# arkworks-rs/pcd

Measured on AMD Instinct MI355X. Metric: msm_mscalar_mul_per_s, higher is better.
Workload: dtype u32 (11 x 28-bit unsaturated Montgomery limbs, v_mad_u64_u32 with 64-bit column accumulators); 1 GPU; MNT4-298 G1 variable-base MSM, n=1048576 pairs per GPU (2^20 per GPU), proving-key bases and scalars resident in HBM, scalar distribution uniform; curve=MNT4-298, group=G1, log_n=20, window_bits=20, windows=15

## Files before the change

### pcd_amd/csrc/ec.hip.h

```cpp
#pragma once
#include <type_traits>
#include "fp.hip.h"

namespace pcd {

template <class F>
struct Jac {
  F X, Y, Z;
  PCD_HD static Jac infinity() { return {F::zero(), F::one(), F::zero()}; }
  PCD_HD bool is_inf() const { return Z.is_zero(); }
  static constexpr int WORDS = 3 * F::WORDS;
  static constexpr int ABI_WORDS = 3 * F::ABI_WORDS;
  PCD_HD static Jac load(const uint32_t* p) { return {F::load(p), F::load(p + F::WORDS), F::load(p + 2 * F::WORDS)}; }
  PCD_HD void store(uint32_t* p) const { X.store(p); Y.store(p + F::WORDS); Z.store(p + 2 * F::WORDS); }
  PCD_HD static Jac from_abi(const uint32_t* w) { return {F::from_abi(w), F::from_abi(w + F::ABI_WORDS), F::from_abi(w + 2 * F::ABI_WORDS)}; }
  PCD_HD void to_abi(uint32_t* w) const { X.to_abi(w); Y.to_abi(w + F::ABI_WORDS); Z.to_abi(w + 2 * F::ABI_WORDS); }
};

template <class F>
struct Aff {
  F x, y;
  static constexpr int WORDS = 2 * F::WORDS;
  static constexpr int ABI_WORDS = 2 * F::ABI_WORDS;
  PCD_HD bool is_inf() const { return x.is_raw_zero() && y.is_raw_zero(); }
// ... 298 lines not shown
    return o;
  }

  struct AccLz {
    typename F::Lz X;
    F Y, ZZ, ZZZ;
    bool inf;
  };
  static constexpr int ACC_WORDS = 4 * F::WORDS;
  PCD_HD static AccLz lz_infinity() { AccLz a; a.X = F::zero().lz(); a.Y = F::one(); a.ZZ = F::zero(); a.ZZZ = F::zero(); a.inf = true; return a; }
  PCD_HD static AccLz lz_from(const J& p) {
    AccLz a;
    a.inf = p.is_inf();
    a.X = p.X.lz(); a.Y = p.Y; a.ZZ = p.Z.sqr(); a.ZZZ = a.ZZ * p.Z;
    return a;
  }
  PCD_HD static J lz_to_jac(const AccLz& a) {
    if (a.inf) return J::infinity();
    return {F::lz_mul(a.X, a.ZZ.lz()), a.Y * a.ZZZ, a.ZZ};
  }
  PCD_HD static AccLz madd_lz(const AccLz& p, const A& q) {
    typedef typename F::Lz L;
    if (q.is_inf()) return p;
    if (p.inf) { AccLz o; o.X = q.x.lz(); o.Y = q.y; o.ZZ = F::one(); o.ZZZ = F::one(); o.inf = false; return o; }
    const L zz = p.ZZ.lz(), zzz = p.ZZZ.lz();
    const F U2 = F::lz_mul(q.x.lz(), zz);
    const F S2 = F::lz_mul(q.y.lz(), zzz);
    const L P = F::lz_carry(F::template lz_sub<2>(U2.lz(), p.X));
    const L R = F::lz_carry(F::template lz_sub<0>(S2.lz(), p.Y.lz()));
    const F PP = F::lz_sqr(P);
    const F RR = F::lz_sqr(R);
    if (PP.is_zero()) {
      if (!RR.is_zero()) return lz_infinity();
      return lz_from(dbl(lz_to_jac(p)));
    }
    const L pp = PP.lz();
    const F PPP = F::lz_mul(P, pp);
    const F Q = F::lz_mul(p.X, pp);
    AccLz o;
    o.inf = false;
    {
      L t;
#pragma unroll
      for (int i = 0; i < F::N; i++)
        t.v[i] = (int32_t)RR.v[i] - (int32_t)PPP.v[i] - (int32_t)(Q.v[i] << 1) + (int32_t)(F::Params::mod4(i) << 1);
      o.X = F::lz_carry(t);
    }
    const L t2 = F::template lz_sub<2>(Q.lz(), o.X);
    const L y1n = F::template lz_sub<0>(F::zero().lz(), p.Y.lz());
    const L ppp = PPP.lz();
    o.Y = F::lz_dot2(R, t2, y1n, ppp);
    o.ZZ = F::lz_mul(zz, pp);
    o.ZZZ = F::lz_mul(zzz, ppp);
    return o;
  }

  template <class ST>
  PCD_HD static void madd_lz_st(ST& st, const A& q) {
    typedef typename F::Lz L;
    if (q.is_inf()) return;
    if (st.inf()) { st.st(0, q.x); st.st(1, q.y); st.st(2, F::one()); st.st(3, F::one()); st.inf() = false; return; }
    auto as_lz = [](const F& f) { L l;
#pragma unroll
      for (int i = 0; i < F::N; i++) l.v[i] = (int32_t)f.v[i];
      return l; };
    auto as_f = [](const L& l) { F f;
#pragma unroll
      for (int i = 0; i < F::N; i++) f.v[i] = (uint32_t)l.v[i];
      return f; };
    const F U2 = F::lz_mul(q.x.lz(), st.ld(2).lz());
    const F S2 = F::lz_mul(q.y.lz(), st.ld(3).lz());
    const L P = F::lz_carry(F::template lz_sub<2>(U2.lz(), as_lz(st.ld(0))));
    const L R = F::lz_carry(F::template lz_sub<0>(S2.lz(), st.ld(1).lz()));
    const F PP = F::lz_sqr(P);
    const F RR = F::lz_sqr(R);
    if (PP.is_zero()) {
      AccLz p;
      p.X = as_lz(st.ld(0)); p.Y = st.ld(1); p.ZZ = st.ld(2); p.ZZZ = st.ld(3); p.inf = false;
      AccLz o = RR.is_zero() ? lz_from(dbl(lz_to_jac(p))) : lz_infinity();
      st.st(0, as_f(o.X)); st.st(1, o.Y); st.st(2, o.ZZ); st.st(3, o.ZZZ); st.inf() = o.inf;
      return;
    }
    const L pp = PP.lz();
    const F PPP = F::lz_mul(P, pp);
    const F Q = F::lz_mul(as_lz(st.ld(0)), pp);
    L x3;
    {
      L t;
#pragma unroll
      for (int i = 0; i < F::N; i++)
        t.v[i] = (int32_t)RR.v[i] - (int32_t)PPP.v[i] - (int32_t)(Q.v[i] << 1) + (int32_t)(F::Params::mod4(i) << 1);
      x3 = F::lz_carry(t);
    }
    const L t2 = F::template lz_sub<2>(Q.lz(), x3);
    st.st(0, as_f(x3));
    const L ppp = PPP.lz();
    {
      const L y1n = F::template lz_sub<0>(F::zero().lz(), st.ld(1).lz());
      st.st(1, F::lz_dot2(R, t2, y1n, ppp));
    }
    st.st(2, F::lz_mul(st.ld(2).lz(), pp));
    st.st(3, F::lz_mul(st.ld(3).lz(), ppp));
  }

  PCD_HD static J mul_w4(const J& p, const uint32_t* k, int nwords, J* table) {
    table[0] = p;
// ... 177 lines not shown
```

### pcd_amd/csrc/fp.hip.h

```cpp
#pragma once
#include <hip/hip_runtime.h>
#include <stdint.h>

#if defined(__HIP_DEVICE_COMPILE__) && !defined(PCD_NO_KEEP_CHAIN)
__device__ __attribute__((weak)) int64_t pcd_never_s = INT64_MIN;
__device__ __attribute__((weak)) uint64_t pcd_never_u = UINT64_MAX;
#define PCD_KEEP_S(acc) __builtin_assume((acc) != pcd_never_s)
#if defined(PCD_KEEP_CHAIN_UNSIGNED)
#define PCD_KEEP_U(acc) __builtin_assume((acc) != pcd_never_u)
#else
#define PCD_KEEP_U(acc) do { if constexpr (N > 11) __builtin_assume((acc) != pcd_never_u); } while (0)
#endif
#if defined(PCD_KEEP_CHAIN_UNSIGNED)
#define PCD_KEEP_UM(acc) __builtin_assume((acc) != pcd_never_u)
#else
#define PCD_KEEP_UM(acc) do { if constexpr (N > 11 && INLINE_ARITH) __builtin_assume((acc) != pcd_never_u); } while (0)
#endif
#else
#define PCD_KEEP_S(acc) ((void)0)
#define PCD_KEEP_U(acc) ((void)0)
#define PCD_KEEP_UM(acc) ((void)0)
#endif


// ... 362 lines not shown
    return r; }
  PCD_HD static Fp lz_dot4(const Lz& a0, const Lz& b0, const Lz& a1, const Lz& b1, const Lz& a2, const Lz& b2, const Lz& a3, const Lz& b3) {
    int32_t m[N];
    int64_t acc = 0;
    PCD_LZ_WIDE_DECL
#pragma unroll
    for (int k = 0; k < N; k++) {
#pragma unroll
      for (int i = 0; i <= k; i++) {
        acc += (int64_t)a0.v[i] * b0.v[k - i]; PCD_KEEP_S(acc); PCD_LZ_WIDE_MAC(a0.v[i], b0.v[k - i])
        acc += (int64_t)a1.v[i] * b1.v[k - i]; PCD_KEEP_S(acc); PCD_LZ_WIDE_MAC(a1.v[i], b1.v[k - i])
        acc += (int64_t)a2.v[i] * b2.v[k - i]; PCD_KEEP_S(acc); PCD_LZ_WIDE_MAC(a2.v[i], b2.v[k - i])
        acc += (int64_t)a3.v[i] * b3.v[k - i]; PCD_KEEP_S(acc); PCD_LZ_WIDE_MAC(a3.v[i], b3.v[k - i])
      }
#pragma unroll
      for (int i = 0; i < k; i++) { acc += (int64_t)m[i] * (int32_t)P::mod(k - i); PCD_KEEP_S(acc); PCD_LZ_WIDE_MAC(m[i], P::mod(k - i)) }
      m[k] = (int32_t)(((uint32_t)acc * P::INV) & MASK);
      acc += (int64_t)m[k] * (int32_t)P::mod(0); PCD_KEEP_S(acc);
      PCD_LZ_WIDE_MAC(m[k], P::mod(0))
      PCD_LZ_WIDE_CHECK();
      acc >>= 28;
    }
    Fp r;
#pragma unroll
    for (int k = N; k < 2 * N - 1; k++) {
#pragma unroll
      for (int i = k - N + 1; i < N; i++) {
        acc += (int64_t)a0.v[i] * b0.v[k - i]; PCD_KEEP_S(acc); PCD_LZ_WIDE_MAC(a0.v[i], b0.v[k - i])
        acc += (int64_t)a1.v[i] * b1.v[k - i]; PCD_KEEP_S(acc); PCD_LZ_WIDE_MAC(a1.v[i], b1.v[k - i])
        acc += (int64_t)a2.v[i] * b2.v[k - i]; PCD_KEEP_S(acc); PCD_LZ_WIDE_MAC(a2.v[i], b2.v[k - i])
        acc += (int64_t)a3.v[i] * b3.v[k - i]; PCD_KEEP_S(acc); PCD_LZ_WIDE_MAC(a3.v[i], b3.v[k - i])
      }
#pragma unroll
      for (int i = k - N + 1; i < N; i++) { acc += (int64_t)m[i] * (int32_t)P::mod(k - i); PCD_KEEP_S(acc); PCD_LZ_WIDE_MAC(m[i], P::mod(k - i)) }
      r.v[k - N] = (uint32_t)acc & MASK;
      PCD_LZ_WIDE_CHECK();
      acc >>= 28;
    }
    if (acc < 0 || acc >= ((int64_t)1 << 28)) {
#if defined(PCD_LZ_CHECK) && !defined(__HIP_DEVICE_COMPILE__)
      abort();
#endif
    }
    r.v[N - 1] = (uint32_t)acc;
    return r;
  }
  PCD_HD static Fp lz_mul(const Lz& a, const Lz& b) { return lz_dot<1>(a, b, a, b); }
  PCD_HD static Fp lz_dot2(const Lz& a0, const Lz& b0, const Lz& a1, const Lz& b1) { return lz_dot<2>(a0, b0, a1, b1); }
  PCD_HD static Fp lz_sqr(const Lz& a) {
    int32_t m[N], a2[N];
#pragma unroll
    for (int i = 0; i < N; i++) a2[i] = a.v[i] * 2;
    int64_t acc = 0;
#pragma unroll
    for (int k = 0; k < N; k++) {
#pragma unroll
      for (int i = 0; 2 * i < k; i++) { acc += (int64_t)a2[i] * a.v[k - i]; PCD_KEEP_S(acc); }
      if ((k & 1) == 0) { acc += (int64_t)a.v[k / 2] * a.v[k / 2]; PCD_KEEP_S(acc); }
#pragma unroll
      for (int i = 0; i < k; i++) { acc += (int64_t)m[i] * (int32_t)P::mod(k - i); PCD_KEEP_S(acc); }
      m[k] = (int32_t)(((uint32_t)acc * P::INV) & MASK);
      acc += (int64_t)m[k] * (int32_t)P::mod(0); PCD_KEEP_S(acc);
      acc >>= 28;
    }
    Fp r;
#pragma unroll
    for (int k = N; k < 2 * N - 1; k++) {
#pragma unroll
      for (int i = k - N + 1; 2 * i < k; i++) { acc += (int64_t)a2[i] * a.v[k - i]; PCD_KEEP_S(acc); }
      if ((k & 1) == 0) { acc += (int64_t)a.v[k / 2] * a.v[k / 2]; PCD_KEEP_S(acc); }
#pragma unroll
      for (int i = k - N + 1; i < N; i++) { acc += (int64_t)m[i] * (int32_t)P::mod(k - i); PCD_KEEP_S(acc); }
      r.v[k - N] = (uint32_t)acc & MASK;
      acc >>= 28;
    }
    r.v[N - 1] = (uint32_t)acc;
    return r;
  }

  template <int TERMS>
  __host__ __device__ __noinline__ static void dot_call(Fp& out, const Fp& a0, const Fp& b0, const Fp& a1, const Fp& b1, const Fp& a2,
                                                        const Fp& b2) {
    dot_impl<TERMS>(out, a0, b0, a1, b1, a2, b2);
  }
  template <int TERMS>
  PCD_HD static void dot(Fp& out, const Fp& a0, const Fp& b0, const Fp& a1, const Fp& b1, const Fp& a2, const Fp& b2) {
    if constexpr (INLINE_ARITH) dot_impl<TERMS>(out, a0, b0, a1, b1, a2, b2); else dot_call<TERMS>(out, a0, b0, a1, b1, a2, b2);
  }
  template <int TERMS>
  PCD_HD static void dot_impl(Fp& out, const Fp& a0, const Fp& b0, const Fp& a1, const Fp& b1, const Fp& a2, const Fp& b2) {
    uint32_t m[N];
    uint64_t acc = 0;
#pragma unroll
    for (int k = 0; k < N; k++) {
#pragma unroll
      for (int i = 0; i <= k; i++) {
        acc += (uint64_t)a0.v[i] * b0.v[k - i]; PCD_KEEP_U(acc);
        acc += (uint64_t)a1.v[i] * b1.v[k - i]; PCD_KEEP_U(acc);
        if (TERMS == 3) { acc += (uint64_t)a2.v[i] * b2.v[k - i]; PCD_KEEP_U(acc); }
      }
#pragma unroll
      for (int i = 0; i < k; i++) { acc += (uint64_t)m[i] * P::mod(k - i); PCD_KEEP_U(acc); }
      m[k] = ((uint32_t)acc * P::INV) & MASK;
      acc += (uint64_t)m[k] * P::mod(0); PCD_KEEP_U(acc);
      acc >>= 28;
    }
    int32_t r[N];
#pragma unroll
    for (int k = N; k < 2 * N - 1; k++) {
#pragma unroll
      for (int i = k - N + 1; i < N; i++) {
        acc += (uint64_t)a0.v[i] * b0.v[k - i]; PCD_KEEP_U(acc);
        acc += (uint64_t)a1.v[i] * b1.v[k - i]; PCD_KEEP_U(acc);
        if (TERMS == 3) { acc += (uint64_t)a2.v[i] * b2.v[k - i]; PCD_KEEP_U(acc); }
      }
#pragma unroll
      for (int i = k - N + 1; i < N; i++) { acc += (uint64_t)m[i] * P::mod(k - i); PCD_KEEP_U(acc); }
      r[k - N] = (int32_t)((uint32_t)acc & MASK);
      acc >>= 28;
    }
    r[N - 1] = (int32_t)(uint32_t)acc;
    if (TERMS == 3) { out = norm_reduce<false>(r); return; }
#pragma unroll
    for (int i = 0; i < N; i++) out.v[i] = (uint32_t)r[i];
  }
  PCD_HD static Fp dot2(const Fp& a0, const Fp& b0, const Fp& a1, const Fp& b1) { Fp o; dot<2>(o, a0, b0, a1, b1, a0, a0); return o; }
// ... 484 lines not shown
```

### pcd_amd/csrc/msm.hip.h

```cpp
#pragma once
#include <cstdlib>
#include <math.h>

#include <algorithm>
#include <atomic>
#include <type_traits>
#include <vector>

#include "ec.hip.h"

namespace pcd {

template <int K>
struct EventSet {
  hipEvent_t e[K] = {};
  bool live = false;
  hipError_t create() {
    for (int i = 0; i < K; i++) { hipError_t r = hipEventCreate(&e[i]); if (r != hipSuccess) return r; }
    live = true;
    return hipSuccess;
  }
  hipEvent_t operator[](int i) const { return e[i]; }
  ~EventSet() { for (int i = 0; i < K; i++) if (e[i]) (void)hipEventDestroy(e[i]); }
};
// ... 668 lines not shown
        w.w = 4 * k + 3 < F::N ? a.v[4 * k + 3] : 0u;
        box[(slot * CH + k) * 64 + threadIdx.x] = w;
      }
    }
  };
  Store s;
  PCD_DEV MsmRunLazyLds() {
    __shared__ V4 accbox[4 * CH * 64];
    s.box = (LdsV4)accbox;
    s.is_inf = true;
  }
  PCD_DEV void add(const Aff<F>& q) { EC<G>::madd_lz_st(s, q); }
  PCD_DEV void flush(uint32_t* dst) {
    if (s.is_inf) { F::zero().store(dst + 2 * F::WORDS); return; }
    s.ld(0).store(dst); s.ld(1).store(dst + F::WORDS); s.ld(2).store(dst + 2 * F::WORDS); s.ld(3).store(dst + 3 * F::WORDS);
    s.is_inf = true;
  }
};
#endif
template <class G, bool XYZZ = MsmUseXyzz<G>::value>
struct MsmStoredPlain {
  typedef typename G::F F;
  static constexpr int WORDS = EC<G>::ACCX_WORDS;
  PCD_DEV static Jac<F> load(const uint32_t* p) {
    typename EC<G>::AccX a = {F::load(p), F::load(p + F::WORDS), F::load(p + 2 * F::WORDS), F::load(p + 3 * F::WORDS)};
    return EC<G>::x_to_jac(a);
  }
  static constexpr bool SEPARATE = true;
};
template <class G>
struct MsmStoredPlain<G, false> {
  typedef typename G::F F;
  static constexpr int WORDS = Jac<F>::WORDS;
  PCD_DEV static Jac<F> load(const uint32_t* p) { return Jac<F>::load(p); }
  static constexpr bool SEPARATE = false;
};
template <class G, bool LAZY = LazyCapable<typename G::F>::value>
struct MsmStored : MsmStoredPlain<G> {};
template <class G>
struct MsmStored<G, true> {
  typedef typename G::F F;
  static constexpr int WORDS = EC<G>::ACC_WORDS;
  PCD_DEV static Jac<F> load(const uint32_t* p) {
    typename EC<G>::AccLz a;
    a.ZZ = F::load(p + 2 * F::WORDS);
    if (a.ZZ.is_zero()) return Jac<F>::infinity();
    a.inf = false;
#pragma unroll
    for (int i = 0; i < F::N; i++) a.X.v[i] = (int32_t)p[i];
    a.Y = F::load(p + F::WORDS);
    a.ZZZ = F::load(p + 3 * F::WORDS);
    return EC<G>::lz_to_jac(a);
  }
  static constexpr bool SEPARATE = true;
};

template <class G>
struct MsmAccWaves {
  typedef typename AccOf<G>::type::F FA;
#ifndef PCD_ACC_WAVES_SPLIT
#define PCD_ACC_WAVES_SPLIT 2
#endif
#ifndef PCD_ACC_WAVES_G1
#define PCD_ACC_WAVES_G1 2
#endif
#ifndef PCD_ACC_WAVES_MB298
#define PCD_ACC_WAVES_MB298 2
#endif
  static constexpr int value = !FA::Base::INLINE_ARITH ? (FA::Base::N <= 11 ? PCD_ACC_WAVES_MB298 : 1)
                             : FA::DEG == 1 ? PCD_ACC_WAVES_G1 : AccOf<G>::LANES > 1 ? PCD_ACC_WAVES_SPLIT : 1;
};

template <class G, bool COMPACT>
__global__ void __launch_bounds__(64, MsmAccWaves<G>::value) msm_accumulate_kernel(const uint32_t* __restrict__ bases, const MsmEntrySource src,
                                                            const uint32_t* __restrict__ off, uint32_t nkeys,
                                                            uint32_t chunk, uint32_t* __restrict__ buckets,
                                                            uint32_t* __restrict__ piece_first, uint32_t* __restrict__ piece_last,
                                                            uint64_t plan ) {
  if (plan) chunk = msm_chunk_of_plan(off[nkeys], plan);
  typedef typename AccOf<G>::type GA;
  typedef typename GA::F F;
  typedef EC<GA> E;
  constexpr int RW = MsmStored<GA>::WORDS;
  constexpr uint32_t LANES = AccOf<G>::LANES, PER_WAVE = 64 / LANES;
  if (threadIdx.x >= PER_WAVE * LANES) return;
  uint32_t t = blockIdx.x * PER_WAVE + threadIdx.x / LANES;
  const uint32_t M = off[nkeys];
  uint64_t start64 = (uint64_t)t * chunk;
  if (start64 >= M) return;
  uint32_t start = (uint32_t)start64, end = (uint32_t)min((uint64_t)M, start64 + chunk);
  if (!COMPACT && src.flag && *src.flag != 0) return;
  if (COMPACT && src.flag && *src.flag == 0) return;
  MsmCursor cur;
  cur.seek(off, nkeys, start);
  bool open_start = cur.key_start < start;
#if PCD_ACC_LDS
  typename std::conditional<LazyCapable<F>::value, MsmRunLazyLds<GA>, MsmRunPlain<GA>>::type acc;
#else
  typename std::conditional<LazyCapable<F>::value, MsmRunLazy<GA>, MsmRunPlain<GA>>::type acc;
#endif
  constexpr bool PREFETCH = F::Base::INLINE_ARITH;
  const uint32_t ones_start = off[src.ones_key];
  auto point_of = [&](uint32_t e) {
    Aff<F> q = Aff<F>::load(bases + (size_t)(e & ~MSM_NEG) * MsmBaseStride<G>::value);
    const F ny = q.y.neg();
    if (e & MSM_NEG) q.y = ny;
    return q;
  };
// ... 284 lines not shown
      for (uint32_t i = 0; i < cnt; i++) {
        const uint32_t k0 = in[(size_t)(2 * i) * 64], l0 = in[(size_t)(2 * i + 1) * 64];
        if (k0 != key) {
          if (open_start) { acc.flush(piece_first + (size_t)t * RW); open_start = false; }
          else acc.flush(buckets + (size_t)key * RW);
          key = k0;
        }
        acc.add(point_of(l0));
      }
      const bool open_end = off[key + 1] > end;
      if (open_end) acc.flush(piece_last + (size_t)t * RW);
      else if (open_start) acc.flush(piece_first + (size_t)t * RW);
      else acc.flush(buckets + (size_t)key * RW);
    }
  }
}

template <class G>
struct MsmItems {
  typedef typename SplitOfTail<G>::type GA;
  static constexpr uint32_t LANES = SplitOfTail<G>::LANES, PER_WAVE = 64 / LANES;
  PCD_DEV static bool idle() { return threadIdx.x >= PER_WAVE * LANES; }
  PCD_DEV static uint32_t local() { return threadIdx.x / LANES; }
  PCD_DEV static uint32_t item() { return blockIdx.x * PER_WAVE + threadIdx.x / LANES; }
  static uint32_t grid(uint32_t items) { return (items + PER_WAVE - 1) / PER_WAVE; }
};

static __global__ void __launch_bounds__(256) msm_zero_kernel(uint32_t* __restrict__ cnt, uint32_t n_cnt, uint32_t* __restrict__ ctl4) {
  const uint32_t i = blockIdx.x * blockDim.x + threadIdx.x;
  if (i < n_cnt) cnt[i] = 0;
  if (i < 4) ctl4[i] = 0;
}

#ifndef PCD_SINGLE_ITEM_PLAIN
#define PCD_SINGLE_ITEM_PLAIN 0
#endif
template <class G> struct MsmSingleItem {
  typedef typename std::conditional<PCD_SINGLE_ITEM_PLAIN != 0, typename SplitOf<G>::type, typename SplitOfTail<G>::type>::type GA;
  static constexpr int LANES = PCD_SINGLE_ITEM_PLAIN != 0 ? SplitOf<G>::LANES : SplitOfTail<G>::LANES;
};
template <class G>
__global__ void __launch_bounds__(64) msm_merge_ones_kernel(uint32_t* __restrict__ buckets, uint32_t ones_key) {
  typedef typename MsmSingleItem<G>::GA GA;
  typedef typename GA::F F;
  if (blockIdx.x != 0 || threadIdx.x >= MsmSingleItem<G>::LANES) return;
  Jac<F> a = Jac<F>::load(buckets + (size_t)1 * Jac<F>::WORDS);
  Jac<F> b = Jac<F>::load(buckets + (size_t)ones_key * Jac<F>::WORDS);
  EC<GA>::add(a, b).store(buckets + (size_t)1 * Jac<F>::WORDS);
}

template <class G>
__global__ void __launch_bounds__(64) msm_fixup_kernel(const uint32_t* __restrict__ off, uint32_t nkeys, const MsmChunkRule rule,
                                                       const uint32_t* __restrict__ piece_first, const uint32_t* __restrict__ piece_last,
                                                       const uint32_t* __restrict__ acc_buckets ,
                                                       uint32_t* __restrict__ buckets, uint32_t big_limit, uint32_t* __restrict__ big_count,
                                                       uint32_t* __restrict__ big_list , uint32_t big_cap,
                                                       uint32_t* __restrict__ seg_list , uint32_t seg_len) {
  const uint32_t chunk = rule.eval(off, nkeys);
  typedef typename MsmItems<G>::GA GA;
  typedef typename GA::F F;
  typedef EC<GA> E;
  constexpr int RW = MsmStored<GA>::WORDS;
  if (MsmItems<G>::idle()) return;
  const bool lead = threadIdx.x % MsmItems<G>::LANES == 0;
  const uint32_t item = MsmItems<G>::item();
  if (item < 2) {
    const uint32_t key = item == 0 ? 1u : nkeys - 1;
    const uint32_t lo = off[key], hi = off[key + 1];
    if (hi == lo) F::zero().store(buckets + (size_t)key * Jac<F>::WORDS + 2 * F::WORDS);
    else if (MsmStored<GA>::SEPARATE && hi - (lo / chunk) * chunk <= chunk)
      MsmStored<GA>::load(acc_buckets + (size_t)key * RW).store(buckets + (size_t)key * Jac<F>::WORDS);
    return;
  }
  const uint32_t t0 = item - 2;
  const uint64_t edge = ((uint64_t)t0 + 1) * chunk;
  if (edge >= off[nkeys]) return;
  const uint32_t key = msm_find_key(off, nkeys, (uint32_t)edge - 1);
  const uint32_t lo = off[key], hi = off[key + 1];
  if (hi <= (uint32_t)edge || lo / chunk != t0) return;
  const uint32_t t1 = (hi - 1) / chunk;
  if (t1 - t0 + 1 > big_limit) {
    if (!lead) return;
    uint32_t nseg = (t1 - t0 + seg_len) / seg_len;
    uint32_t slot = atomicAdd(&big_count[0], 1u);
    uint32_t s0 = atomicAdd(&big_count[1], nseg);
    if (slot < big_cap) { big_list[3 * slot] = key; big_list[3 * slot + 1] = s0; big_list[3 * slot + 2] = nseg; }
    for (uint32_t i = 0; i < nseg; i++) {
      uint32_t lo = t0 + i * seg_len, hi = min(t1, lo + seg_len - 1);
      seg_list[3 * (s0 + i)] = lo; seg_list[3 * (s0 + i) + 1] = hi; seg_list[3 * (s0 + i) + 2] = t1;
    }
    return;
  }
  Jac<F> acc = MsmStored<GA>::load(piece_last + (size_t)t0 * RW);
  for (uint32_t u = t0 + 1; u < t1; u++) acc = E::add(acc, MsmStored<GA>::load(piece_last + (size_t)u * RW));
  acc = E::add(acc, MsmStored<GA>::load(piece_first + (size_t)t1 * RW));
  acc.store(buckets + (size_t)key * Jac<F>::WORDS);
}

template <class G, bool ENABLE = true, bool Q = true>
struct MsmPairItems {
  static constexpr bool TWO = ENABLE && TwoLaneOps<G>::value && (MsmItems<G>::LANES == 1 || HalfLanes<typename MsmItems<G>::GA::F>::L == (int)MsmItems<G>::LANES);
  static constexpr bool QUAD = Q && TWO && MsmItems<G>::LANES == 1 && PCD_EC4 != 0;
  static constexpr uint32_t BASE = MsmItems<G>::LANES, LANES = QUAD ? 4 : TWO ? 2 * BASE : BASE, PER_WAVE = 64 / LANES;
  PCD_DEV static bool idle() { return threadIdx.x >= PER_WAVE * LANES; }
  PCD_DEV static uint32_t item() { return blockIdx.x * PER_WAVE + threadIdx.x / LANES; }
  PCD_DEV static uint32_t local() { return threadIdx.x / LANES; }
  PCD_DEV static bool writer() { return QUAD ? (threadIdx.x & 3u) == 0 : (!TWO || (((threadIdx.x & 63u) / BASE) & 1u) == 0); }
  static uint32_t grid(uint32_t items) { return (items + PER_WAVE - 1) / PER_WAVE; }
};
template <class G, bool TWO = MsmPairItems<G, true>::TWO, bool Q = true>
struct MsmPairOps {
  typedef typename MsmItems<G>::GA GA;
  typedef Jac<typename GA::F> J;
  PCD_DEV static J add(const J& a, const J& b) { return EC<GA>::add(a, b); }
  PCD_DEV static J dbl(const J& a) { return EC<GA>::dbl(a); }
};
template <class G, bool Q>
struct MsmPairOps<G, true, Q> {
  typedef typename SplitOfTail<G>::type GA;
  typedef Jac<typename GA::F> J;
  PCD_DEV static J add(const J& a, const J& b) { if constexpr (MsmPairItems<G, true, Q>::QUAD) return EC4<GA>::add4(a, b); else return EC2<GA>::add2(a, b); }
  PCD_DEV static J dbl(const J& a) { if constexpr (MsmPairItems<G, true, Q>::QUAD) return EC4<GA>::dbl4(a); else return EC2<GA>::dbl2(a); }
};
template <class G>
PCD_DEV void msm_wave_tree(Jac<typename MsmPairOps<G>::GA::F> acc, uint32_t* my , uint32_t* dst) {
  typedef MsmPairItems<G> IT;
  typedef MsmPairOps<G> O;
  typedef typename O::GA::F F;
  constexpr uint32_t PW = IT::PER_WAVE;
  const uint32_t it = IT::local();
  const bool live = !IT::idle();
  if (live && IT::writer()) acc.store(my + (size_t)it * Jac<F>::WORDS);
  __syncthreads();
  for (uint32_t s = 32; s > 0; s >>= 1) {
    if (live && it < s && it + s < PW) {
      Jac<F> o = Jac<F>::load(my + (size_t)(it + s) * Jac<F>::WORDS);
      acc = O::add(acc, o);
      if (IT::writer()) acc.store(my + (size_t)it * Jac<F>::WORDS);
    }
    __syncthreads();
  }
  if (live && it == 0 && IT::writer()) acc.store(dst);
  __syncthreads();
}
template <class G>
__global__ void __launch_bounds__(64) msm_big_segments_kernel(const uint32_t* __restrict__ seg_list, const uint32_t* __restrict__ big_count,
                                                              const uint32_t* __restrict__ piece_first, const uint32_t* __restrict__ piece_last,
                                                              uint32_t* __restrict__ partial, uint32_t* __restrict__ scratch) {
  typedef MsmPairItems<G> IT;
  typedef MsmPairOps<G> O;
  typedef typename O::GA GA;
  typedef typename GA::F F;
  constexpr uint32_t PW = IT::PER_WAVE;
  const uint32_t nseg = big_count[1];
  uint32_t* my = scratch + (size_t)blockIdx.x * 64 * Jac<F>::WORDS;
  for (uint32_t sg = blockIdx.x; sg < nseg; sg += gridDim.x) {
    uint32_t lo = seg_list[3 * sg], hi = seg_list[3 * sg + 1], tlast = seg_list[3 * sg + 2];
    Jac<F> acc = Jac<F>::infinity();
    if (!IT::idle())
      for (uint32_t u = lo + IT::local(); u <= hi; u += PW) {
        const uint32_t* src = (u == tlast) ? piece_first : piece_last;
        acc = O::add(acc, MsmStored<GA>::load(src + (size_t)u * MsmStored<GA>::WORDS));
      }
    msm_wave_tree<G>(acc, my, partial + (size_t)sg * Jac<F>::WORDS);
  }
}
template <class G>
__global__ void __launch_bounds__(64) msm_big_bucket_kernel(const uint32_t* __restrict__ big_list, const uint32_t* __restrict__ big_count,
                                                            const uint32_t* __restrict__ partial, uint32_t* __restrict__ buckets,
                                                            uint32_t* __restrict__ scratch) {
  typedef MsmPairItems<G> IT;
  typedef MsmPairOps<G> O;
  typedef typename O::GA GA;
  typedef typename GA::F F;
  constexpr uint32_t PW = IT::PER_WAVE;
  const uint32_t nbig = big_count[0];
  uint32_t* my = scratch + (size_t)blockIdx.x * 64 * Jac<F>::WORDS;
  for (uint32_t b = blockIdx.x; b < nbig; b += gridDim.x) {
    uint32_t key = big_list[3 * b], s0 = big_list[3 * b + 1], ns = big_list[3 * b + 2];
    Jac<F> acc = Jac<F>::infinity();
    if (!IT::idle())
      for (uint32_t u = IT::local(); u < ns; u += PW) acc = O::add(acc, Jac<F>::load(partial + (size_t)(s0 + u) * Jac<F>::WORDS));
    msm_wave_tree<G>(acc, my, buckets + (size_t)key * Jac<F>::WORDS);
  }
}

struct MsmBucketSrc {
  const uint32_t* off;
  const uint32_t* acc_buckets;
  const uint32_t* buckets;
  uint32_t nkeys;
  MsmChunkRule rule;
};
template <class GA>
PCD_DEV Jac<typename GA::F> msm_bucket_at(const MsmBucketSrc& bs, uint32_t chunk, uint32_t key) {
  typedef typename GA::F F;
  if (key != 1) {
    const uint32_t lo = bs.off[key], hi = bs.off[key + 1];
    if (hi == lo) return Jac<F>::infinity();
    if (hi - (lo / chunk) * chunk <= chunk)
      return MsmStored<GA>::load(bs.acc_buckets + (size_t)key * MsmStored<GA>::WORDS);
  }
  return Jac<F>::load(bs.buckets + (size_t)key * Jac<F>::WORDS);
}
template <class G, bool WIDE>
__global__ void __launch_bounds__(64) msm_tail_level_kernel(const MsmBucketSrc bs, uint32_t mA, size_t strideA_in,
                                                            const uint32_t* __restrict__ C_in, uint32_t mC, size_t strideC_in,
                                                            uint32_t* __restrict__ A_out, size_t strideA_out,
                                                            uint32_t* __restrict__ C_out, size_t strideC_out, int k) {
  typedef MsmPairItems<G, WIDE> IT;
  typedef MsmPairOps<G, IT::TWO> O;
  typedef typename O::GA GA;
  typedef typename GA::F F;
  constexpr int PW = Jac<F>::WORDS;
  if (IT::idle()) return;
  uint32_t K = 1u << k;
  uint32_t JA = (mA + K - 1) >> k, JC = (mC + K - 1) >> k;
  uint32_t tid = IT::item();
  uint32_t w = blockIdx.y;
  if (tid < JA) {
    const uint32_t chunk = bs.rule.eval(bs.off, bs.nkeys);
    const uint32_t key1 = w * (uint32_t)strideA_in + 1;
    Jac<F> run = Jac<F>::infinity(), acc = Jac<F>::infinity();
    for (int tt = (int)K - 1; tt >= 0; tt--) {
      uint32_t i = tid * K + tt;
      if (i < mA) run = O::add(run, msm_bucket_at<GA>(bs, chunk, key1 + i));
      acc = O::add(acc, run);
    }
    if (IT::writer()) acc.store(C_out + (w * strideC_out + JC + tid) * PW);
    if (tid >= 1) {
      for (int d = 0; d < k; d++) run = O::dbl(run);
      if (IT::writer()) run.store(A_out + (w * strideA_out + tid - 1) * PW);
    }
  } else if (tid < JA + JC) {
    uint32_t j = tid - JA;
    const uint32_t* Cw = C_in + w * strideC_in * PW;
    Jac<F> acc = Jac<F>::infinity();
    for (uint32_t tt = 0; tt < K; tt++) {
      uint32_t i = j * K + tt;
      if (i < mC) acc = O::add(acc, Jac<F>::load(Cw + (size_t)i * PW));
    }
    if (IT::writer()) acc.store(C_out + (w * strideC_out + j) * PW);
  }
}

template <class G, bool Q = true, bool FIRST = false>
PCD_DEV void msm_tail_pair_item(int role, uint32_t j, uint32_t w, const uint32_t* A_in, uint32_t mA, size_t strideA_in, const uint32_t* C_in,
                                uint32_t mC, size_t strideC_in, uint32_t* A_out, size_t strideA_out, uint32_t* C_out, size_t strideC_out,
                                const MsmBucketSrc* bs = nullptr) {
  typedef MsmPairOps<G, MsmPairItems<G, true>::TWO, Q> O;
  typedef typename O::GA GA;
  typedef typename GA::F F;
  typedef MsmPairItems<G, true, Q> IT;
  constexpr int PW = Jac<F>::WORDS;
  const uint32_t JA = (mA + 1) >> 1, JC = (mC + 1) >> 1;
  if (role < 2) {
    if (j >= JA) return;
    uint32_t chunk = 0;
    if constexpr (FIRST) chunk = bs->rule.eval(bs->off, bs->nkeys);
    auto a_at = [&](uint32_t i) {
      if constexpr (FIRST) return msm_bucket_at<GA>(*bs, chunk, w * (uint32_t)strideA_in + 1 + i);
      else return Jac<F>::load(A_in + (w * strideA_in + i) * PW);
    };
    const bool two = 2 * j + 1 < mA;
    const Jac<F> a0 = a_at(2 * j);
    if (role == 0) {
      if (j == 0) return;
      Jac<F> run = two ? O::add(a0, a_at(2 * j + 1)) : a0;
      run = O::dbl(run);
      if (IT::writer()) run.store(A_out + (w * strideA_out + j - 1) * PW);
    } else {
      Jac<F> acc = two ? O::add(O::dbl(a_at(2 * j + 1)), a0) : a0;
      if (IT::writer()) acc.store(C_out + (w * strideC_out + JC + j) * PW);
    }
  } else {
    if (j >= JC) return;
    const uint32_t* Cw = C_in + w * strideC_in * PW;
    Jac<F> acc = Jac<F>::load(Cw + (size_t)(2 * j) * PW);
    if (2 * j + 1 < mC) acc = O::add(acc, Jac<F>::load(Cw + (size_t)(2 * j + 1) * PW));
    if (IT::writer()) acc.store(C_out + (w * strideC_out + j) * PW);
  }
}
template <class G, bool Q = true>
__global__ void __launch_bounds__(64) msm_tail_pair_kernel(const uint32_t* __restrict__ A_in, uint32_t mA, size_t strideA_in,
                                                           const uint32_t* __restrict__ C_in, uint32_t mC, size_t strideC_in,
                                                           uint32_t* __restrict__ A_out, size_t strideA_out,
                                                           uint32_t* __restrict__ C_out, size_t strideC_out) {
  typedef MsmPairItems<G, true, Q> IT;
  if (IT::idle()) return;
  msm_tail_pair_item<G, Q>((int)blockIdx.z, IT::item(), blockIdx.y, A_in, mA, strideA_in, C_in, mC, strideC_in, A_out, strideA_out, C_out, strideC_out);
}
template <class G, bool Q = true>
__global__ void __launch_bounds__(64) msm_tail_pair_first_kernel(const MsmBucketSrc bs, uint32_t mA, size_t strideA_in,
                                                                 uint32_t* __restrict__ A_out, size_t strideA_out,
                                                                 uint32_t* __restrict__ C_out, size_t strideC_out) {
  typedef MsmPairItems<G, true, Q> IT;
  if (IT::idle()) return;
  msm_tail_pair_item<G, Q, true>((int)blockIdx.z, IT::item(), blockIdx.y, nullptr, mA, strideA_in, nullptr, 0u, 0, A_out, strideA_out, C_out, strideC_out, &bs);
}
constexpr uint32_t MSM_FUSED_WAVES = 4;
#ifndef PCD_QUAD_MAX_ITEMS
#define PCD_QUAD_MAX_ITEMS 4096
#endif
constexpr uint32_t MSM_QUAD_MAX_ITEMS = PCD_QUAD_MAX_ITEMS;
template <class G>
struct MsmFusedTail {
  static constexpr bool ENABLED = !MsmPairOps<G>::GA::F::Base::MAILBOX;
  static uint32_t waves(uint32_t items) { return (items + MsmPairItems<G>::PER_WAVE - 1) / MsmPairItems<G>::PER_WAVE; }
  static bool fits(uint32_t mA, uint32_t mC) { return ENABLED && 2 * waves((mA + 1) >> 1) + waves((mC + 1) >> 1) <= MSM_FUSED_WAVES; }
};
template <class G>
__global__ void __launch_bounds__(64 * MSM_FUSED_WAVES) msm_tail_fused_kernel(const uint32_t* A_in, uint32_t mA, size_t strideA_in, const uint32_t* C_in,
// ... 372 lines not shown
  hipStream_t own = st;
  if (lane) {
    if (!ws.lane_in) PCD_HIP_TRY(hipEventCreateWithFlags(&ws.lane_in, hipEventDisableTiming));
    if (!ws.lane_out) PCD_HIP_TRY(hipEventCreateWithFlags(&ws.lane_out, hipEventDisableTiming));
    PCD_HIP_TRY(hipEventRecord(ws.lane_in, own));
    PCD_HIP_TRY(hipStreamWaitEvent(lane->stream, ws.lane_in, 0));
    st = lane->stream;
  }
  {
    constexpr uint32_t per_wave = 64 / AccOf<G>::LANES;
    const dim3 acc_grid((nchunks + per_wave - 1) / per_wave);
    bool launched = false;
    if constexpr (MsmTreeCapable<G>::value) {
      if (use_tree) {
        constexpr int FW = AccOf<G>::type::F::WORDS;
        const uint32_t grid = tree_grid;
        MsmTreeBufs tb;
        tb.cap = tree_cap;
        tb.phases = 3;
        uint32_t* chunk_word = big_count + 2;
        hipLaunchKernelGGL(msm_tree_plan_kernel, dim3(1), dim3(1), 0, st, off, tkeys, grid * 64, tree_cap, tree_chunk, chunk_word);
        tree_chunk_dev = chunk_word;
        PCD_HIP_TRY(ws.ensure(WS_TLIST, MsmTreeBufs::list_words(tb.cap) * 4 * grid));
        PCD_HIP_TRY(ws.ensure(WS_TPAIR, MsmTreeBufs::pair_words(tb.cap) * 4 * grid));
        PCD_HIP_TRY(ws.ensure(WS_TPREFIX, MsmTreeBufs::prefix_words(tb.cap, FW) * 4 * grid));
        PCD_HIP_TRY(ws.ensure(WS_TPTS, MsmTreeBufs::pts_words(tb.cap, FW) * 4 * grid));
        tb.list = (uint32_t*)ws.buf[WS_TLIST]; tb.pairs = (uint32_t*)ws.buf[WS_TPAIR];
        tb.prefix = (uint32_t*)ws.buf[WS_TPREFIX]; tb.pts = (uint32_t*)ws.buf[WS_TPTS];
        hipLaunchKernelGGL((msm_pair_tree_kernel<G>), dim3(grid), dim3(64), 0, st, bases_dev, src, off, tkeys, chunk_word, tb,
                           tree_min_pairs ? tree_min_pairs : MSM_TREE_MIN_PAIRS, acc_buckets, pfirst, plast);
        launched = true;
      }
    }
    if (!launched) {
      if (src.slots) hipLaunchKernelGGL((msm_accumulate_kernel<G, false>), acc_grid, dim3(64), 0, st, bases_dev, src, off, tkeys, pl.chunk, acc_buckets, pfirst, plast, plan_word);
      hipLaunchKernelGGL((msm_accumulate_kernel<G, true>), acc_grid, dim3(64), 0, st, bases_dev, src, off, tkeys, pl.chunk, acc_buckets, pfirst, plast, plan_word);
    }
  }
  if (lane) {
    PCD_HIP_TRY(hipEventRecord(ws.lane_out, st));
    st = own;
    PCD_HIP_TRY(hipStreamWaitEvent(st, ws.lane_out, 0));
  }
  PCD_HIP_TRY(mark(4));
  const MsmChunkRule chunk_rule = {tree_chunk_dev, plan_word, pl.chunk};
  hipLaunchKernelGGL((msm_fixup_kernel<G>), dim3(MsmItems<G>::grid(nchunks + 2)), dim3(64), 0, st, off, tkeys, chunk_rule, pfirst, plast, acc_buckets,
                     buckets, big_limit, big_count, big, big_cap, seg_list, seg_len);
  {
    const uint32_t big_grid = std::min<uint32_t>(seg_cap, 2048);
    PCD_HIP_TRY(ws.ensure(WS_BIGSCR, (size_t)big_grid * 64 * PB));
    hipLaunchKernelGGL((msm_big_segments_kernel<G>), dim3(big_grid), dim3(64), 0, st, seg_list, big_count, pfirst, plast, big_partial,
                       (uint32_t*)ws.buf[WS_BIGSCR]);
    hipLaunchKernelGGL((msm_big_bucket_kernel<G>), dim3(std::min<uint32_t>(big_cap, 2048)), dim3(64), 0, st, big, big_count, big_partial,
                       buckets, (uint32_t*)ws.buf[WS_BIGSCR]);
  }
  hipLaunchKernelGGL((msm_merge_ones_kernel<G>), dim3(1), dim3(64), 0, st, buckets, ones_key);
  PCD_HIP_TRY(mark(5));
  {
    const uint32_t B = 1u << (pl.c - 1);
    size_t cap_pts = ((size_t)1 << pl.c);
    PCD_HIP_TRY(ws.ensure(WS_A0, (size_t)Wg * cap_pts * PB / 2 + PB * Wg * 4));
    PCD_HIP_TRY(ws.ensure(WS_A1, (size_t)Wg * cap_pts * PB / 2 + PB * Wg * 4));
    PCD_HIP_TRY(ws.ensure(WS_C0, (size_t)Wg * cap_pts * PB / 2 + PB * Wg * 4));
    PCD_HIP_TRY(ws.ensure(WS_C1, (size_t)Wg * cap_pts * PB / 2 + PB * Wg * 4));
    const size_t strideAC = cap_pts / 2 + 4;
    const MsmBucketSrc bucket_src = {off, acc_buckets, buckets, tkeys, chunk_rule};
    const uint32_t* A_in = buckets + PW;
    size_t strideA_in = (size_t)1 << pl.c;
    const uint32_t* C_in = nullptr;
    size_t strideC_in = 0;
    uint32_t mA = B, mC = 0;
    int flip = 0, level = 0;
    bool fused = false;
    while (mA > 0 || mC > 1) {
      int k = (level == 0 && B >= (1u << 17)) ? 3 : 1;
      uint32_t K = 1u << k;
      uint32_t JA = (mA + K - 1) >> k, JC = (mC + K - 1) >> k;
      uint32_t* A_out = (uint32_t*)ws.buf[flip ? WS_A1 : WS_A0];
      uint32_t* C_out = (uint32_t*)ws.buf[flip ? WS_C1 : WS_C0];
      uint32_t threads = JA + JC;
      if (!fused && level > 0 && MsmFusedTail<G>::fits(mA, mC)) {
        hipLaunchKernelGGL((msm_tail_fused_kernel<G>), dim3(Wg), dim3(64 * MSM_FUSED_WAVES), 0, st, A_in, mA, strideA_in, C_in, mC, strideC_in,
                           (uint32_t*)ws.buf[WS_A0], (uint32_t*)ws.buf[WS_A1], (uint32_t*)ws.buf[WS_C0], (uint32_t*)ws.buf[WS_C1], strideAC, flip);
        fused = true;
      }
      if (fused) {
      } else if (level == 0 && k == 1 && JA * (uint32_t)Wg > MSM_QUAD_MAX_ITEMS)
        hipLaunchKernelGGL((msm_tail_pair_first_kernel<G, false>), dim3(MsmPairItems<G, true, false>::grid(JA), Wg, 2), dim3(64), 0, st, bucket_src, mA,
                           strideA_in, A_out, strideAC, C_out, strideAC);
      else if (level == 0 && k == 1)
        hipLaunchKernelGGL((msm_tail_pair_first_kernel<G>), dim3(MsmPairItems<G>::grid(JA), Wg, 2), dim3(64), 0, st, bucket_src, mA, strideA_in, A_out,
                           strideAC, C_out, strideAC);
      else if (k == 1 && std::max(JA, JC) * (uint32_t)Wg > MSM_QUAD_MAX_ITEMS)
        hipLaunchKernelGGL((msm_tail_pair_kernel<G, false>), dim3(MsmPairItems<G, true, false>::grid(std::max(JA, JC)), Wg, 3), dim3(64), 0, st, A_in, mA,
                           strideA_in, C_in, mC, strideC_in, A_out, strideAC, C_out, strideAC);
      else if (k == 1)
        hipLaunchKernelGGL((msm_tail_pair_kernel<G>), dim3(MsmPairItems<G>::grid(std::max(JA, JC)), Wg, 3), dim3(64), 0, st, A_in, mA, strideA_in, C_in,
                           mC, strideC_in, A_out, strideAC, C_out, strideAC);
      else if (threads <= (1u << 15))
        hipLaunchKernelGGL((msm_tail_level_kernel<G, true>), dim3(MsmPairItems<G, true>::grid(threads), Wg), dim3(64), 0, st, bucket_src, mA, strideA_in, C_in,
                           mC, strideC_in, A_out, strideAC, C_out, strideAC, k);
      else
        hipLaunchKernelGGL((msm_tail_level_kernel<G, false>), dim3(MsmPairItems<G, false>::grid(threads), Wg), dim3(64), 0, st, bucket_src, mA, strideA_in, C_in,
                           mC, strideC_in, A_out, strideAC, C_out, strideAC, k);
      mA = JA ? JA - 1 : 0;
      mC = JC + JA;
      A_in = A_out; strideA_in = strideAC;
// ... 23 lines not shown
```

Baseline: 427.4 Mscalar-mul/s.

## Keep bucket epilogue in lazy XYZZ form instead of converting to Jacobian

Adds an XYZZ-coordinate add_lz on lazy-reduced limbs and uses it in the fixup kernel and the first tail level, so partial bucket sums stay in lazy XYZZ form and are written back to acc_buckets. Jacobian conversion is deferred until the bucket is consumed, and the per-bucket chunk rule evaluation in msm_bucket_at goes away. Large buckets also record their XYZZ result. The aim is to avoid repeated Jacobian conversions and costlier Jacobian adds, at the price of a general XYZZ add that needs extra multiplies for ZZ/ZZZ. lz_sqr also gains wide-check instrumentation hooks.

```diff
diff --git a/pcd_amd/csrc/ec.hip.h b/pcd_amd/csrc/ec.hip.h
--- a/pcd_amd/csrc/ec.hip.h
+++ b/pcd_amd/csrc/ec.hip.h
@@ -374,6 +374,43 @@
     o.Y = F::lz_dot2(R, t2, y1n, ppp);
     o.ZZ = F::lz_mul(zz, pp);
     o.ZZZ = F::lz_mul(zzz, ppp);
+    return o;
+  }
+
+  PCD_HD static AccLz add_lz(const AccLz& p, const AccLz& q) {
+    typedef typename F::Lz L;
+    if (p.inf) return q;
+    if (q.inf) return p;
+    const F U1 = F::lz_mul(p.X, q.ZZ.lz());
+    const F U2 = F::lz_mul(q.X, p.ZZ.lz());
+    const F S1 = F::lz_mul(p.Y.lz(), q.ZZZ.lz());
+    const F S2 = F::lz_mul(q.Y.lz(), p.ZZZ.lz());
+    const L P = F::lz_carry(F::template lz_sub<0>(U2.lz(), U1.lz()));
+    const L R = F::lz_carry(F::template lz_sub<0>(S2.lz(), S1.lz()));
+    const F PP = F::lz_sqr(P);
+    const F RR = F::lz_sqr(R);
+    if (PP.is_zero()) {
+      if (!RR.is_zero()) return lz_infinity();
+      return lz_from(dbl(lz_to_jac(p)));
+    }
+    const L pp = PP.lz();
+    const F PPP = F::lz_mul(P, pp);
+    const F Q = F::lz_mul(U1.lz(), pp);
+    AccLz o;
+    o.inf = false;
+    {
+      L t;
+#pragma unroll
+      for (int i = 0; i < F::N; i++)
+        t.v[i] = (int32_t)RR.v[i] - (int32_t)PPP.v[i] - (int32_t)(Q.v[i] << 1) + (int32_t)(F::Params::mod4(i) << 1);
+      o.X = F::lz_carry(t);
+    }
+    const L t2 = F::template lz_sub<2>(Q.lz(), o.X);
+    const L s1n = F::template lz_sub<0>(F::zero().lz(), S1.lz());
+    const L ppp = PPP.lz();
+    o.Y = F::lz_dot2(R, t2, s1n, ppp);
+    o.ZZ = F::lz_mul(F::lz_mul(p.ZZ.lz(), q.ZZ.lz()).lz(), pp);
+    o.ZZZ = F::lz_mul(F::lz_mul(p.ZZZ.lz(), q.ZZZ.lz()).lz(), ppp);
     return o;
   }
 
diff --git a/pcd_amd/csrc/fp.hip.h b/pcd_amd/csrc/fp.hip.h
--- a/pcd_amd/csrc/fp.hip.h
+++ b/pcd_amd/csrc/fp.hip.h
@@ -438,26 +438,30 @@
 #pragma unroll
     for (int i = 0; i < N; i++) a2[i] = a.v[i] * 2;
     int64_t acc = 0;
+    PCD_LZ_WIDE_DECL
 #pragma unroll
     for (int k = 0; k < N; k++) {
 #pragma unroll
-      for (int i = 0; 2 * i < k; i++) { acc += (int64_t)a2[i] * a.v[k - i]; PCD_KEEP_S(acc); }
-      if ((k & 1) == 0) { acc += (int64_t)a.v[k / 2] * a.v[k / 2]; PCD_KEEP_S(acc); }
-#pragma unroll
-      for (int i = 0; i < k; i++) { acc += (int64_t)m[i] * (int32_t)P::mod(k - i); PCD_KEEP_S(acc); }
+      for (int i = 0; 2 * i < k; i++) { acc += (int64_t)a2[i] * a.v[k - i]; PCD_KEEP_S(acc); PCD_LZ_WIDE_MAC(a2[i], a.v[k - i]) }
+      if ((k & 1) == 0) { acc += (int64_t)a.v[k / 2] * a.v[k / 2]; PCD_KEEP_S(acc); PCD_LZ_WIDE_MAC(a.v[k / 2], a.v[k / 2]) }
+#pragma unroll
+      for (int i = 0; i < k; i++) { acc += (int64_t)m[i] * (int32_t)P::mod(k - i); PCD_KEEP_S(acc); PCD_LZ_WIDE_MAC(m[i], P::mod(k - i)) }
       m[k] = (int32_t)(((uint32_t)acc * P::INV) & MASK);
       acc += (int64_t)m[k] * (int32_t)P::mod(0); PCD_KEEP_S(acc);
+      PCD_LZ_WIDE_MAC(m[k], P::mod(0))
+      PCD_LZ_WIDE_CHECK();
       acc >>= 28;
     }
     Fp r;
 #pragma unroll
     for (int k = N; k < 2 * N - 1; k++) {
 #pragma unroll
-      for (int i = k - N + 1; 2 * i < k; i++) { acc += (int64_t)a2[i] * a.v[k - i]; PCD_KEEP_S(acc); }
-      if ((k & 1) == 0) { acc += (int64_t)a.v[k / 2] * a.v[k / 2]; PCD_KEEP_S(acc); }
-#pragma unroll
-      for (int i = k - N + 1; i < N; i++) { acc += (int64_t)m[i] * (int32_t)P::mod(k - i); PCD_KEEP_S(acc); }
+      for (int i = k - N + 1; 2 * i < k; i++) { acc += (int64_t)a2[i] * a.v[k - i]; PCD_KEEP_S(acc); PCD_LZ_WIDE_MAC(a2[i], a.v[k - i]) }
+      if ((k & 1) == 0) { acc += (int64_t)a.v[k / 2] * a.v[k / 2]; PCD_KEEP_S(acc); PCD_LZ_WIDE_MAC(a.v[k / 2], a.v[k / 2]) }
+#pragma unroll
+      for (int i = k - N + 1; i < N; i++) { acc += (int64_t)m[i] * (int32_t)P::mod(k - i); PCD_KEEP_S(acc); PCD_LZ_WIDE_MAC(m[i], P::mod(k - i)) }
       r.v[k - N] = (uint32_t)acc & MASK;
+      PCD_LZ_WIDE_CHECK();
       acc >>= 28;
     }
     r.v[N - 1] = (uint32_t)acc;
diff --git a/pcd_amd/csrc/msm.hip.h b/pcd_amd/csrc/msm.hip.h
--- a/pcd_amd/csrc/msm.hip.h
+++ b/pcd_amd/csrc/msm.hip.h
@@ -744,8 +744,31 @@
     a.ZZZ = F::load(p + 3 * F::WORDS);
     return EC<G>::lz_to_jac(a);
   }
+  PCD_DEV static typename EC<G>::AccLz load_lz(const uint32_t* p) {
+    typename EC<G>::AccLz a;
+#pragma unroll
+    for (int i = 0; i < F::N; i++) a.X.v[i] = (int32_t)p[i];
+    a.Y = F::load(p + F::WORDS);
+    a.ZZ = F::load(p + 2 * F::WORDS);
+    a.ZZZ = F::load(p + 3 * F::WORDS);
+    a.inf = a.ZZ.is_zero();
+    return a;
+  }
+  PCD_DEV static void store_lz(const typename EC<G>::AccLz& a, uint32_t* dst) {
+    if (a.inf) { F::zero().store(dst + 2 * F::WORDS); return; }
+#pragma unroll
+    for (int i = 0; i < F::N; i++) dst[i] = (uint32_t)a.X.v[i];
+    a.Y.store(dst + F::WORDS);
+    a.ZZ.store(dst + 2 * F::WORDS);
+    a.ZZZ.store(dst + 3 * F::WORDS);
+  }
   static constexpr bool SEPARATE = true;
 };
+#ifndef PCD_EPILOGUE_LZ
+#define PCD_EPILOGUE_LZ 1
+#endif
+template <class G>
+struct MsmEpilogueLz { static constexpr bool value = PCD_EPILOGUE_LZ != 0 && LazyCapable<typename G::F>::value; };
 
 template <class G>
 struct MsmAccWaves {
@@ -1136,7 +1159,7 @@
 template <class G>
 __global__ void __launch_bounds__(64) msm_fixup_kernel(const uint32_t* __restrict__ off, uint32_t nkeys, const MsmChunkRule rule,
                                                        const uint32_t* __restrict__ piece_first, const uint32_t* __restrict__ piece_last,
-                                                       const uint32_t* __restrict__ acc_buckets ,
+                                                       uint32_t* acc_buckets ,
                                                        uint32_t* __restrict__ buckets, uint32_t big_limit, uint32_t* __restrict__ big_count,
                                                        uint32_t* __restrict__ big_list , uint32_t big_cap,
                                                        uint32_t* __restrict__ seg_list , uint32_t seg_len) {
@@ -1175,10 +1198,19 @@
     }
     return;
   }
-  Jac<F> acc = MsmStored<GA>::load(piece_last + (size_t)t0 * RW);
-  for (uint32_t u = t0 + 1; u < t1; u++) acc = E::add(acc, MsmStored<GA>::load(piece_last + (size_t)u * RW));
-  acc = E::add(acc, MsmStored<GA>::load(piece_first + (size_t)t1 * RW));
-  acc.store(buckets + (size_t)key * Jac<F>::WORDS);
+  if constexpr (MsmEpilogueLz<GA>::value) {
+    typedef MsmStored<GA> S;
+    typename E::AccLz acc = S::load_lz(piece_last + (size_t)t0 * RW);
+    for (uint32_t u = t0 + 1; u < t1; u++) acc = E::add_lz(acc, S::load_lz(piece_last + (size_t)u * RW));
+    acc = E::add_lz(acc, S::load_lz(piece_first + (size_t)t1 * RW));
+    if (key == 1 || key == nkeys - 1) E::lz_to_jac(acc).store(buckets + (size_t)key * Jac<F>::WORDS);
+    else S::store_lz(acc, acc_buckets + (size_t)key * RW);
+  } else {
+    Jac<F> acc = MsmStored<GA>::load(piece_last + (size_t)t0 * RW);
+    for (uint32_t u = t0 + 1; u < t1; u++) acc = E::add(acc, MsmStored<GA>::load(piece_last + (size_t)u * RW));
+    acc = E::add(acc, MsmStored<GA>::load(piece_first + (size_t)t1 * RW));
+    acc.store(buckets + (size_t)key * Jac<F>::WORDS);
+  }
 }
 
 template <class G, bool ENABLE = true, bool Q = true>
@@ -1207,7 +1239,8 @@
   PCD_DEV static J dbl(const J& a) { if constexpr (MsmPairItems<G, true, Q>::QUAD) return EC4<GA>::dbl4(a); else return EC2<GA>::dbl2(a); }
 };
 template <class G>
-PCD_DEV void msm_wave_tree(Jac<typename MsmPairOps<G>::GA::F> acc, uint32_t* my , uint32_t* dst) {
+PCD_DEV void msm_wave_tree(Jac<typename MsmPairOps<G>::GA::F> acc, uint32_t* my , uint32_t* dst,
+                           uint32_t* dst_record = nullptr ) {
   typedef MsmPairItems<G> IT;
   typedef MsmPairOps<G> O;
   typedef typename O::GA::F F;
@@ -1224,7 +1257,14 @@
     }
     __syncthreads();
   }
-  if (live && it == 0 && IT::writer()) acc.store(dst);
+  if (live && it == 0 && IT::writer()) {
+    if constexpr (MsmEpilogueLz<typename O::GA>::value) {
+      if (dst_record) MsmStored<typename O::GA>::store_lz(EC<typename O::GA>::lz_from(acc), dst_record);
+      else acc.store(dst);
+    } else {
+      acc.store(dst);
+    }
+  }
   __syncthreads();
 }
 template <class G>
@@ -1252,7 +1292,9 @@
 template <class G>
 __global__ void __launch_bounds__(64) msm_big_bucket_kernel(const uint32_t* __restrict__ big_list, const uint32_t* __restrict__ big_count,
                                                             const uint32_t* __restrict__ partial, uint32_t* __restrict__ buckets,
-                                                            uint32_t* __restrict__ scratch) {
+                                                            uint32_t* __restrict__ scratch,
+                                                            uint32_t* acc_buckets ,
+                                                            uint32_t nkeys) {
   typedef MsmPairItems<G> IT;
   typedef MsmPairOps<G> O;
   typedef typename O::GA GA;
@@ -1265,7 +1307,10 @@
     Jac<F> acc = Jac<F>::infinity();
     if (!IT::idle())
       for (uint32_t u = IT::local(); u < ns; u += PW) acc = O::add(acc, Jac<F>::load(partial + (size_t)(s0 + u) * Jac<F>::WORDS));
-    msm_wave_tree<G>(acc, my, buckets + (size_t)key * Jac<F>::WORDS);
+    uint32_t* rec = nullptr;
+    if constexpr (MsmEpilogueLz<GA>::value)
+      if (key != 1 && key != nkeys - 1) rec = acc_buckets + (size_t)key * MsmStored<GA>::WORDS;
+    msm_wave_tree<G>(acc, my, buckets + (size_t)key * Jac<F>::WORDS, rec);
   }
 }
 
@@ -1279,13 +1324,27 @@
 template <class GA>
 PCD_DEV Jac<typename GA::F> msm_bucket_at(const MsmBucketSrc& bs, uint32_t chunk, uint32_t key) {
   typedef typename GA::F F;
-  if (key != 1) {
-    const uint32_t lo = bs.off[key], hi = bs.off[key + 1];
-    if (hi == lo) return Jac<F>::infinity();
-    if (hi - (lo / chunk) * chunk <= chunk)
-      return MsmStored<GA>::load(bs.acc_buckets + (size_t)key * MsmStored<GA>::WORDS);
-  }
-  return Jac<F>::load(bs.buckets + (size_t)key * Jac<F>::WORDS);
+  if constexpr (MsmEpilogueLz<GA>::value) {
+    if (key == 1) return Jac<F>::load(bs.buckets + (size_t)key * Jac<F>::WORDS);
+    if (bs.off[key + 1] == bs.off[key]) return Jac<F>::infinity();
+    return MsmStored<GA>::load(bs.acc_buckets + (size_t)key * MsmStored<GA>::WORDS);
+  } else {
+    if (key != 1) {
+      const uint32_t lo = bs.off[key], hi = bs.off[key + 1];
+      if (hi == lo) return Jac<F>::infinity();
+      if (hi - (lo / chunk) * chunk <= chunk)
+        return MsmStored<GA>::load(bs.acc_buckets + (size_t)key * MsmStored<GA>::WORDS);
+    }
+    return Jac<F>::load(bs.buckets + (size_t)key * Jac<F>::WORDS);
+  }
+}
+template <class GA>
+PCD_DEV typename EC<GA>::AccLz msm_bucket_lz(const MsmBucketSrc& bs, uint32_t key) {
+  typedef typename GA::F F;
+  if (key == 1) return EC<GA>::lz_from(Jac<F>::load(bs.buckets + (size_t)key * Jac<F>::WORDS));
+  typename EC<GA>::AccLz a = MsmStored<GA>::load_lz(bs.acc_buckets + (size_t)key * MsmStored<GA>::WORDS);
+  a.inf = a.inf || bs.off[key + 1] == bs.off[key];
+  return a;
 }
 template <class G, bool WIDE>
 __global__ void __launch_bounds__(64) msm_tail_level_kernel(const MsmBucketSrc bs, uint32_t mA, size_t strideA_in,
@@ -1303,13 +1362,26 @@
   uint32_t tid = IT::item();
   uint32_t w = blockIdx.y;
   if (tid < JA) {
-    const uint32_t chunk = bs.rule.eval(bs.off, bs.nkeys);
     const uint32_t key1 = w * (uint32_t)strideA_in + 1;
     Jac<F> run = Jac<F>::infinity(), acc = Jac<F>::infinity();
-    for (int tt = (int)K - 1; tt >= 0; tt--) {
-      uint32_t i = tid * K + tt;
-      if (i < mA) run = O::add(run, msm_bucket_at<GA>(bs, chunk, key1 + i));
-      acc = O::add(acc, run);
+    if constexpr (MsmEpilogueLz<GA>::value && !IT::TWO) {
+      typedef EC<GA> E;
+      typename E::AccLz run_lz = E::lz_infinity(), acc_lz = E::lz_infinity();
+      for (int tt = (int)K - 1; tt >= 0; tt--) {
+        uint32_t i = tid * K + tt;
+        if (i < mA) run_lz = E::add_lz(run_lz, msm_bucket_lz<GA>(bs, key1 + i));
+        acc_lz = E::add_lz(acc_lz, run_lz);
+      }
+      run = E::lz_to_jac(run_lz);
+      acc = E::lz_to_jac(acc_lz);
+    } else {
+      uint32_t chunk = 0;
+      if constexpr (!MsmEpilogueLz<GA>::value) chunk = bs.rule.eval(bs.off, bs.nkeys);
+      for (int tt = (int)K - 1; tt >= 0; tt--) {
+        uint32_t i = tid * K + tt;
+        if (i < mA) run = O::add(run, msm_bucket_at<GA>(bs, chunk, key1 + i));
+        acc = O::add(acc, run);
+      }
     }
     if (IT::writer()) acc.store(C_out + (w * strideC_out + JC + tid) * PW);
     if (tid >= 1) {
@@ -1341,7 +1413,7 @@
   if (role < 2) {
     if (j >= JA) return;
     uint32_t chunk = 0;
-    if constexpr (FIRST) chunk = bs->rule.eval(bs->off, bs->nkeys);
+    if constexpr (FIRST && !MsmEpilogueLz<GA>::value) chunk = bs->rule.eval(bs->off, bs->nkeys);
     auto a_at = [&](uint32_t i) {
       if constexpr (FIRST) return msm_bucket_at<GA>(*bs, chunk, w * (uint32_t)strideA_in + 1 + i);
       else return Jac<F>::load(A_in + (w * strideA_in + i) * PW);
@@ -1820,7 +1892,7 @@
     hipLaunchKernelGGL((msm_big_segments_kernel<G>), dim3(big_grid), dim3(64), 0, st, seg_list, big_count, pfirst, plast, big_partial,
                        (uint32_t*)ws.buf[WS_BIGSCR]);
     hipLaunchKernelGGL((msm_big_bucket_kernel<G>), dim3(std::min<uint32_t>(big_cap, 2048)), dim3(64), 0, st, big, big_count, big_partial,
-                       buckets, (uint32_t*)ws.buf[WS_BIGSCR]);
+                       buckets, (uint32_t*)ws.buf[WS_BIGSCR], acc_buckets, tkeys);
   }
   hipLaunchKernelGGL((msm_merge_ones_kernel<G>), dim3(1), dim3(64), 0, st, buckets, ones_key);
   PCD_HIP_TRY(mark(5));
```

Result: faster. 444.4 Mscalar-mul/s (median of 6 runs) (+4.0%).
